# maturk/dn-splatter

Hardware: AMD Instinct MI355X
Metric: fwd+bwd frames/sec @1M Gaussians 1080p; HBM GB/s vs roofline (higher is better)
Workload: dtype f32; 1 GPU; c2: 1000000 random-init Gaussians, 1 camera/GPU 1920x1080, SH degree 3 + expected depth + per-Gaussian normals (7 channels, fused one-pass, post-ops in HIP), fx=fy=1200.0, orbit r=8, closed-form 3-NN scale init, random dense cotangents; scene=reference_init, N=1000000, pixels=2073600, bin_policy=deferred, parallelism=single GPU

## Files before the change

dn-splatter_amd/csrc/binning.hip:

```cpp

#include <assert.h>
#include <string.h>
#include "splat_common.h"
#include "bin_ranges.h"
#include "depth_buckets.h"

namespace {

constexpr int RS_THREADS = 256;
#ifndef DNS_RS_ITEMS_I
#define DNS_RS_ITEMS_I 16
#endif
constexpr int RS_ITEMS_I = DNS_RS_ITEMS_I;
#ifndef DNS_RS_ITEMS_N
#define DNS_RS_ITEMS_N 8
#endif
constexpr int RS_ITEMS_N = DNS_RS_ITEMS_N;
constexpr int RS_ITEMS_N_LARGE = 2 * DNS_RS_ITEMS_N;
constexpr int RS_LARGE_N = 1 << 22;
inline int rs_items_n(int N) { return N >= RS_LARGE_N ? RS_ITEMS_N_LARGE : RS_ITEMS_N; }
#ifndef DNS_TI_THREADS
#define DNS_TI_THREADS 512
#endif
constexpr int TI_THREADS = DNS_TI_THREADS;
// ... 28 lines not shown
#pragma unroll
    for (int i = 0; i < NW; ++i) {
        uint32_t s = lds_wave[i];
        if (i < w) base += s;
        tot += s;
    }
    total = tot;
    __syncthreads();
    return inc + base;
}
__device__ __forceinline__ uint32_t block_incl_scan_256(uint32_t v, uint32_t *lds_wave , uint32_t &total)
{
    return block_incl_scan<4>(v, lds_wave, total);
}

__device__ __forceinline__ uint32_t depth_key(const int32_t *__restrict__ radii, const float *__restrict__ depths, uint32_t g)
{
    return radii[g] > 0 ? __float_as_uint(depths[g]) : 0xFFFFFFFFu;
}

struct __align__(16) EmitRec {
    uint32_t gid;
    uint32_t start;
    uint32_t base_tile;
    uint32_t bw;
};
struct GenArgs {
    const EmitRec *__restrict__ jrec;
    const uint32_t *__restrict__ cum;
    const uint32_t *__restrict__ chunk_first;
// ... 128 lines not shown
                k[i] = __float_as_uint(depths[idc]);
                ok[i] = ok[i] && r > 0;
            } else k[i] = (uint32_t)keys[idc];
        }
#pragma unroll
        for (int i = 0; i < ITEMS; ++i)
            if (ok[i]) atomicAdd(&hist[(k[i] >> shift) & mask], 1u);
    }
    __syncthreads();
    if (threadIdx.x <= mask) table[(size_t)threadIdx.x * nb + blockIdx.x] = hist[threadIdx.x];
}

#ifndef DNS_GEN_HIST_RANGES
#define DNS_GEN_HIST_RANGES 1
#endif
template <int ITEMS, int TH>
__global__ __launch_bounds__(TH) void radix_hist_ranges_kernel(const uint32_t *__restrict__ n_ptr, uint32_t n_cap, int dbits,
                                                               uint32_t *__restrict__ table, int nb, int32_t *__restrict__ tile_first,
                                                               int n_tiles, int32_t *__restrict__ tile_end, GenArgs gen,
                                                               uint32_t *__restrict__ status)
{
    __shared__ uint32_t diff[RS_DIGITS + 1];
    __shared__ uint32_t all_s;
    __shared__ uint32_t lds_wave[TH / DNS_WAVE];
    static_assert(TH > RS_DIGITS, "one thread per difference slot");
    const uint32_t n = n_ptr ? min(*n_ptr, n_cap) : n_cap;
    if (tile_first)
        for (int i = blockIdx.x * TH + threadIdx.x; i <= n_tiles; i += gridDim.x * TH) tile_first[i] = (int32_t)n;
    if (tile_end)
        for (int i = blockIdx.x * TH + threadIdx.x; i < n_tiles; i += gridDim.x * TH) tile_end[i] = 0;
    if (status && blockIdx.x == 0 && threadIdx.x == 0) *status = 0u;
    const uint32_t ND = 1u << dbits;
    if (threadIdx.x <= ND) diff[threadIdx.x] = 0u;
    if (threadIdx.x == 0) all_s = 0u;
    __syncthreads();
    const uint32_t q0 = blockIdx.x * (uint32_t)(TH * ITEMS);
    if (q0 < n) {
        const uint32_t q1 = q0 + min((uint32_t)(TH * ITEMS), n - q0);
        const uint32_t j0 = gen.chunk_first[blockIdx.x];
        const uint32_t n_ranked = min(*gen.n_ranked, (uint32_t)gen.N);
        uint32_t all = 0u;
        for (uint32_t jb = j0;; jb += TH) {
            const uint32_t jj = jb + threadIdx.x;
            bool inside = false;
            if (jj < n_ranked) {
                const uint32_t e = gen.cum[jj], s = jj ? gen.cum[jj - 1] : 0u;
                inside = s < q1;
                if (inside && e > s && e > q0) {
                    const uint4 r = *reinterpret_cast<const uint4 *>(gen.jrec + jj);
                    all += dns_record_digit_ranges(r.z, r.w, (uint32_t)gen.tw, max(s, q0) - s, min(e, q1) - s, dbits,
                                                   [&](uint32_t d0, uint32_t len) {
                                                       atomicAdd(&diff[d0], 1u);
                                                       const uint32_t end = d0 + len;
                                                       if (end <= ND) atomicAdd(&diff[end], 0xFFFFFFFFu);
                                                       else { atomicAdd(&diff[0], 1u); atomicAdd(&diff[end - ND], 0xFFFFFFFFu); }
                                                   });
                }
            }
            if (!__syncthreads_or(inside && threadIdx.x == TH - 1)) break;
        }
        if (all) atomicAdd(&all_s, all);
    }
    __syncthreads();
    const uint32_t v = threadIdx.x < ND ? diff[threadIdx.x] : 0u;
    uint32_t tot;
    const uint32_t inc = block_incl_scan<TH / DNS_WAVE>(v, lds_wave, tot);
    if (threadIdx.x < ND) table[(size_t)threadIdx.x * nb + blockIdx.x] = inc + all_s;
}

constexpr int SC_MAX_SEGS = 8;
__global__ __launch_bounds__(SC_THREADS) void radix_scan_kernel(uint32_t *__restrict__ table, int nb, uint32_t *__restrict__ segsum,
                                                                int segs, int seg_len)
{
    __shared__ uint32_t lds_wave[4];
    const int d = blockIdx.x / segs, sgm = blockIdx.x - d * segs;
    uint32_t *row = table + (size_t)d * nb;
    const int lo = sgm * seg_len, hi = min(nb, lo + seg_len);
    uint32_t carry = 0;
    for (int start = lo; start < hi; start += SC_CHUNK) {
        const int i0 = start + threadIdx.x * SC_ITEMS;
        uint32_t v[SC_ITEMS];
        uint32_t s = 0;
// ... 170 lines not shown
        int2 bx[ITEMS];
#pragma unroll
        for (int r = 0; r < ITEMS; ++r) {
            const uint32_t i = min((uint32_t)(r * TH + threadIdx.x), n_out - 1u);
            const uint32_t d = ((uint32_t)keys_s[i] >> shift) & DMASK;
            dsts[r] = gbase[d] + (i - dstart[d]);
            vs[r] = vals_s[i];
        }
#pragma unroll
        for (int r = 0; r < ITEMS; ++r) bx[r] = box_in[vs[r]];
#pragma unroll
        for (int r = 0; r < ITEMS; ++r)
            if ((uint32_t)(r * TH + threadIdx.x) < n_out) {
                vals_out[dsts[r]] = vs[r];
                box_out[dsts[r]] = bx[r];
                tiles_out[dsts[r]] = ((uint32_t)bx[r].y & 0xffffu) * ((uint32_t)bx[r].y >> 16);
            }
        return;
    }
#pragma unroll
    for (int r = 0; r < ITEMS; ++r) {
        const uint32_t i = r * TH + threadIdx.x;
        if (i < n_out) {
            const uint32_t k = keys_s[i];
            const uint32_t d = (k >> shift) & DMASK;
            const uint32_t dst = gbase[d] + (i - dstart[d]);
            if (!LAST) keys_out[dst] = (K)k;
            vals_out[dst] = vals_s[i];
            if (LAST && (i == 0 || (uint32_t)keys_s[i - 1] != k)) atomicMin(&tile_first[k], (int32_t)dst);
            if (LAST && tile_end && (i + 1 == n_valid || (uint32_t)keys_s[i + 1] != k)) atomicMax(&tile_end[k], (int32_t)dst + 1);
        }
// ... 44 lines not shown
        uint32_t k[U];
#pragma unroll
        for (int u = 0; u < U; ++u) {
            const uint32_t i = min(i0 + u * DP_THREADS, n - 1u);
            r[u] = radii[i];
            k[u] = __float_as_uint(depths[i]);
        }
#pragma unroll
        for (int u = 0; u < U; ++u)
            if (r[u] > 0) { mn = min(mn, k[u]); mx = max(mx, k[u]); }
    }
    dp_block_minmax(mn, mx, red);
    if (threadIdx.x == 0) { part[2 * blockIdx.x] = mn; part[2 * blockIdx.x + 1] = mx; }
}

template <int BBITS>
__global__ __launch_bounds__(DP_THREADS) void depth_part_hist_kernel(const int32_t *__restrict__ radii, const float *__restrict__ depths,
                                                                     uint32_t n, const uint32_t *__restrict__ part, int n_part,
                                                                     uint32_t *__restrict__ ks, uint32_t *__restrict__ table, int nb,
                                                                     int sub)
{
    constexpr int NB = 1 << BBITS;
    __shared__ uint32_t hist[NB];
    __shared__ uint32_t red[2 * DP_NW];
    uint32_t mn = 0xFFFFFFFFu, mx = 0u;
    for (int i = threadIdx.x; i < n_part; i += DP_THREADS) { mn = min(mn, part[2 * i]); mx = max(mx, part[2 * i + 1]); }
    for (int d = threadIdx.x; d < NB; d += DP_THREADS) hist[d] = 0u;
    dp_block_minmax(mn, mx, red);
    uint32_t kmin = 0u;
    int shift = 0;
    if (mn <= mx) { kmin = mn; shift = dns_depth_bucket_shift(mn, mx, BBITS); }
    if (blockIdx.x == 0 && threadIdx.x == 0) { ks[0] = kmin; ks[1] = (uint32_t)shift; }
    for (int c = 0; c < sub; ++c) {
        const uint32_t base = (blockIdx.x * sub + c) * DP_CHUNK;
        if (base >= n) break;
        int32_t r[DP_ITEMS];
        uint32_t k[DP_ITEMS];
#pragma unroll
        for (int i = 0; i < DP_ITEMS; ++i) {
            const uint32_t idc = min(base + i * DP_THREADS + threadIdx.x, n - 1u);
            r[i] = radii[idc];
            k[i] = __float_as_uint(depths[idc]);
        }
#pragma unroll
        for (int i = 0; i < DP_ITEMS; ++i)
            if (base + i * DP_THREADS + threadIdx.x < n && r[i] > 0) atomicAdd(&hist[dns_depth_bucket(k[i], kmin, shift) & (NB - 1)], 1u);
    }
    __syncthreads();
    for (int d = threadIdx.x; d < NB; d += DP_THREADS) table[(size_t)d * nb + blockIdx.x] = hist[d];
}

template <int BBITS>
__global__ __launch_bounds__(DP_THREADS) void depth_part_scatter_kernel(
    const int32_t *__restrict__ radii, const float *__restrict__ depths, uint32_t n, const uint32_t *__restrict__ ks,
    uint2 *__restrict__ pairs_out, const uint32_t *__restrict__ table, const uint32_t *__restrict__ totals, int nb, int segs, int seg_len,
    uint32_t *__restrict__ count_out, uint32_t *__restrict__ bucket_start, int sub)
{
    constexpr int NB = 1 << BBITS;
    constexpr int DPT = NB / DP_THREADS;
    static_assert(NB % DP_THREADS == 0 && DP_CHUNK <= 0xFFFF, "bucket scan layout / 16-bit chunk-local counts");
    __shared__ __align__(4) uint16_t wave_cnt[DP_NW][NB];
    __shared__ uint32_t gbase[NB];
    __shared__ uint32_t lds_wave[DP_NW];
    const uint32_t base0 = blockIdx.x * sub * DP_CHUNK;
    if (base0 >= n) return;
    const uint32_t kmin = ks[0];
    const int shift = (int)ks[1];
    const int w = threadIdx.x / DNS_WAVE;
    const uint32_t lane = lane_id();
    const uint64_t lt_mask = (lane == 0) ? 0ull : (~0ull >> (64 - lane));
    {
// ... 11 lines not shown
                if (sg < my_seg) pre_tab[q] += v;
            }
            tsum += pre_tot[q];
        }
        uint32_t total;
        const uint32_t inc = block_incl_scan<DP_NW>(tsum, lds_wave, total);
        uint32_t run = inc - tsum;
#pragma unroll
        for (int q = 0; q < DPT; ++q) {
            const int d = threadIdx.x * DPT + q;
            gbase[d] = run + pre_tab[q];
            if (blockIdx.x == 0) bucket_start[d] = run;
            run += pre_tot[q];
        }
        if (blockIdx.x == 0 && threadIdx.x == 0) { bucket_start[NB] = total; *count_out = total; }
    }
    for (int c = 0; c < sub; ++c) {
        const uint32_t base = base0 + c * DP_CHUNK;
        if (base >= n) break;
        {
            uint32_t *z = reinterpret_cast<uint32_t *>(&wave_cnt[0][0]);
            for (int i = threadIdx.x; i < DP_NW * NB / 2; i += DP_THREADS) z[i] = 0u;
        }
        __syncthreads();
        const uint32_t wave_start = base + w * (DNS_WAVE * DP_ITEMS);
        uint32_t key[DP_ITEMS];
        int32_t rad[DP_ITEMS];
        uint16_t rnk[DP_ITEMS];
#pragma unroll
        for (int r = 0; r < DP_ITEMS; ++r) {
// ... 90 lines not shown
            for (int q = 0; q < DP_NW; ++q)
                if (q < w) pos += wave_cnt[q][d];
            dst[pos] = p;
        }
        __syncthreads();
        {
            uint32_t s = 0u;
#pragma unroll
            for (int q = 0; q < DP_NW; ++q) { s += wave_cnt[q][threadIdx.x]; wave_cnt[q][threadIdx.x] = 0u; }
            dig_run[threadIdx.x] += s;
        }
        __syncthreads();
    }
}

__device__ __forceinline__ void dp_store_bucket(const uint2 *res, uint32_t s, uint32_t n, uint32_t *__restrict__ vals_out,
                                                const int2 *__restrict__ box_in, int2 *__restrict__ box_out,
                                                uint32_t *__restrict__ tiles_out)
{
    constexpr int U = 4;
    for (uint32_t i0 = threadIdx.x; i0 < n; i0 += U * DP_THREADS) {
        uint32_t v[U];
        int2 bx[U];
#pragma unroll
        for (int u = 0; u < U; ++u) v[u] = res[min(i0 + u * DP_THREADS, n - 1u)].y;
        if (box_in) {
#pragma unroll
            for (int u = 0; u < U; ++u) bx[u] = box_in[v[u]];
        }
#pragma unroll
        for (int u = 0; u < U; ++u) {
            const uint32_t i = i0 + u * DP_THREADS;
            if (i < n) {
                vals_out[s + i] = v[u];
                if (box_in) {
                    box_out[s + i] = bx[u];
                    tiles_out[s + i] = ((uint32_t)bx[u].y & 0xffffu) * ((uint32_t)bx[u].y >> 16);
                }
            }
        }
    }
}

__device__ __forceinline__ void dp_sort_in_lds(const uint2 *__restrict__ in, uint32_t n, uint32_t kmin, int passes, int dbits, uint2 *buf,
                                               uint32_t *dig_start , uint32_t (*wave_cnt)[256] , uint32_t *lds_wave)
{
    constexpr int ITEMS = DP_CAP / DP_THREADS;
    const int w = threadIdx.x / DNS_WAVE;
    const uint32_t lane = lane_id();
    const uint64_t lt_mask = (lane == 0) ? 0ull : (~0ull >> (64 - lane));
    const int ipw = (int)((n + DP_THREADS - 1) / DP_THREADS);
    const uint32_t first = (uint32_t)w * DNS_WAVE * ipw + lane;
    const uint32_t mask = (1u << dbits) - 1u;
    uint2 p[ITEMS];
    uint32_t rnk[ITEMS];
// ... 45 lines not shown
        for (int r = 0; r < ITEMS; ++r)
            if (r < ipw && first + r * DNS_WAVE < n) {
                const uint32_t d = ((p[r].x - kmin) >> sh) & mask;
                buf[dig_start[d] + wave_cnt[w][d] + rnk[r]] = p[r];
            }
        __syncthreads();
        if (pass + 1 < passes) {
#pragma unroll
            for (int r = 0; r < ITEMS; ++r)
                if (r < ipw) p[r] = buf[min(first + r * DNS_WAVE, n - 1u)];
        }
    }
    __syncthreads();
}

__global__ __launch_bounds__(DP_THREADS) void depth_bucket_sort_kernel(const uint32_t *__restrict__ ks,
                                                                       const uint32_t *__restrict__ bucket_start, uint2 *pairs_a,
                                                                       uint2 *pairs_b, uint32_t *__restrict__ vals_out,
                                                                       const int2 *__restrict__ box_in, int2 *__restrict__ box_out,
                                                                       uint32_t *__restrict__ tiles_out)
{
    __shared__ uint2 buf[DP_CAP];
    __shared__ uint32_t dig_run[256];
    __shared__ uint32_t wave_cnt[DP_NW][256];
    __shared__ uint32_t lds_wave[DP_NW];
    const uint32_t s = bucket_start[blockIdx.x], n = bucket_start[blockIdx.x + 1] - s;
    if (n == 0) return;
    const uint32_t kmin = ks[0];
    const int shift = (int)ks[1];
    const int passes = dns_depth_local_passes(shift), dbits = dns_depth_local_bits(shift);
    if (n <= (uint32_t)DP_CAP) {
        dp_sort_in_lds(pairs_a + s, n, kmin, passes, dbits, buf, dig_run, wave_cnt, lds_wave);
        dp_store_bucket(buf, s, n, vals_out, box_in, box_out, tiles_out);
    } else {
        uint2 *src = pairs_a + s, *dst = pairs_b + s;
        for (int p = 0; p < passes; ++p) {
            dp_lsd_pass(src, dst, n, kmin, p * dbits, dbits, dig_run, wave_cnt, lds_wave);
            uint2 *t = src; src = dst; dst = t;
        }
        dp_store_bucket(src, s, n, vals_out, box_in, box_out, tiles_out);
    }
}

template <bool BOXES>
__global__ __launch_bounds__(SC_THREADS) void scan_sums_kernel(int N, const uint32_t *__restrict__ n_ptr,
                                                               const uint32_t *__restrict__ order,
                                                               const int32_t *__restrict__ tiles,
                                                               uint32_t *__restrict__ sums, uint32_t *__restrict__ tiles_sorted,
                                                               const int2 *__restrict__ boxes = nullptr,
                                                               int2 *__restrict__ boxes_sorted = nullptr)
{
    __shared__ uint32_t lds_wave[4];
    const int n = (int)min(*n_ptr, (uint32_t)N);
    const int base = blockIdx.x * SC_CHUNK + threadIdx.x * SC_ITEMS;
    uint32_t s = 0;
    if (blockIdx.x * SC_CHUNK < n) {
        uint32_t o[SC_ITEMS], t[SC_ITEMS];
        [[maybe_unused]] int2 bx[SC_ITEMS];
#pragma unroll
        for (int i = 0; i < SC_ITEMS; ++i) o[i] = order[min(base + i, n - 1)];
#pragma unroll
        for (int i = 0; i < SC_ITEMS; ++i) {
            if (BOXES) {
                bx[i] = boxes[o[i]];
                t[i] = ((uint32_t)bx[i].y & 0xffffu) * ((uint32_t)bx[i].y >> 16);
            } else t[i] = (uint32_t)tiles[o[i]];
        }
#pragma unroll
        for (int i = 0; i < SC_ITEMS; ++i)
            if (base + i < n) {
                s += t[i];
                tiles_sorted[base + i] = t[i];
                if (BOXES) boxes_sorted[base + i] = bx[i];
            }
    }
    uint32_t tot;
    block_incl_scan_256(s, lds_wave, tot);
    if (threadIdx.x == 0) sums[blockIdx.x] = tot;
}

__global__ __launch_bounds__(SC_THREADS) void scan_sums_sorted_kernel(int N, const uint32_t *__restrict__ n_ptr,
                                                                      const uint32_t *__restrict__ tiles_sorted, uint32_t *__restrict__ sums)
{
    __shared__ uint32_t lds_wave[4];
    const int n = (int)min(*n_ptr, (uint32_t)N);
    const int base = blockIdx.x * SC_CHUNK + threadIdx.x * SC_ITEMS;
    uint32_t s = 0;
#pragma unroll
    for (int i = 0; i < SC_ITEMS; ++i)
        if (base + i < n) s += tiles_sorted[base + i];
    uint32_t tot;
    block_incl_scan_256(s, lds_wave, tot);
    if (threadIdx.x == 0) sums[blockIdx.x] = tot;
}

struct EmitPrep {
    EmitRec *__restrict__ jrec;
    uint32_t *__restrict__ chunk_first;
    int nb_chunks, chunk;
    int n_per_cam, tile_size, tw, th;
    const float *__restrict__ means2d;
    const int32_t *__restrict__ radii;
    const float4 *__restrict__ splats;
    const int2 *__restrict__ boxes;
    const int2 *__restrict__ boxes_sorted;
};

__device__ __forceinline__ void emit_record(const EmitPrep &ep, int N, uint32_t j, uint32_t gid, uint32_t start, uint32_t end)
{
    EmitRec r;
    r.gid = gid; r.start = start;
    const uint32_t cam_tiles = (ep.n_per_cam < N) ? (gid / (uint32_t)ep.n_per_cam) * (uint32_t)(ep.tw * ep.th) : 0u;
    if (ep.boxes) {
        const int2 b = ep.boxes_sorted ? ep.boxes_sorted[j] : ep.boxes[gid];
        r.bw = (uint32_t)b.y & 0xffffu;
        r.base_tile = (uint32_t)b.x + cam_tiles;
    } else {
        int x0, y0, x1, y1;
        if (ep.splats) {
            const float4 r0 = ep.splats[(size_t)gid * 4], r1 = ep.splats[(size_t)gid * 4 + 1];
            dns_snug_tile_bbox(r0.x, r0.y, r0.z, r0.w, r1.x, r1.y, (float)ep.radii[gid], ep.tile_size, ep.tw, ep.th, x0, y0, x1, y1);
        } else
            dns_tile_bbox(ep.means2d[2 * gid], ep.means2d[2 * gid + 1], (float)ep.radii[gid], ep.tile_size, ep.tw, ep.th, x0, y0, x1, y1);
        r.base_tile = (uint32_t)(y0 * ep.tw + x0) + cam_tiles;
        r.bw = (uint32_t)(x1 - x0);
    }
    ep.jrec[j] = r;
    const uint32_t c_lo = (start + (uint32_t)ep.chunk - 1u) / (uint32_t)ep.chunk, c_hi = (end - 1u) / (uint32_t)ep.chunk;
    for (uint32_t c = c_lo; c <= c_hi && c < (uint32_t)ep.nb_chunks; ++c) ep.chunk_first[c] = j;
}

__global__ __launch_bounds__(SC_THREADS) void scan_final_kernel(int N, const uint32_t *__restrict__ n_ptr,
                                                                const uint32_t *__restrict__ order,
                                                                const int32_t *__restrict__ tiles,
                                                                const uint32_t *__restrict__ sums,
                                                                uint32_t *__restrict__ cum, uint32_t *__restrict__ total_u32,
                                                                int64_t *__restrict__ total_i64, int64_t *__restrict__ total_max)
{
    __shared__ uint32_t lds_wave[4];
    const int n = (int)min(*n_ptr, (uint32_t)N);
    if (n == 0 && blockIdx.x == 0 && threadIdx.x == 0) { *total_u32 = 0u; *total_i64 = 0; }
    if (blockIdx.x * SC_CHUNK >= n) return;
    const int base = blockIdx.x * SC_CHUNK + threadIdx.x * SC_ITEMS;
    uint32_t v[SC_ITEMS];
// ... 82 lines not shown
    uint32_t *key_a, *key_b, *val_a, *val_b;
    uint32_t *cum;
    uint32_t *tiles_sorted;
    int2 *boxes_sorted;
    EmitRec *jrec;
    uint32_t *chunk_first;
    uint32_t *tab_n;
    uint32_t *totals;
    uint32_t *sums;
    uint32_t *total;
    uint32_t *status;
    uint32_t *n_ranked;
    uint32_t *dp_part;
    uint32_t *dp_ks;
    uint32_t *dp_start;
    uint32_t *dp_tab;
    uint32_t *dp_totals;
    uint32_t *tkey_b, *tval_b;
    uint32_t *tkey_c, *tval_c;
    uint32_t *tab_i;
    int nb_n, nb_i, nb_scan, nb_p;
    size_t bytes;
};

inline size_t align_up(size_t v, size_t a) { return (v + a - 1) / a * a; }

BinWs carve(void *ws, int N, int64_t cap)
{
    BinWs b{};
    b.nb_n = (N + RS_THREADS * rs_items_n(N) - 1) / (RS_THREADS * rs_items_n(N));
    b.nb_i = (int)((cap + RS_THREADS * RS_ITEMS_I - 1) / (RS_THREADS * RS_ITEMS_I));
    b.nb_scan = (N + SC_CHUNK - 1) / SC_CHUNK;
// ... 11 lines not shown
    };
    size_t n = (size_t)(N > 0 ? N : 1), c = (size_t)(cap > 0 ? cap : 1);
    b.key_a = take(n); b.key_b = take(n); b.val_a = take(n); b.val_b = take(n);
    b.cum = take(n);
    b.tiles_sorted = take(n);
    b.boxes_sorted = reinterpret_cast<int2 *>(take(2 * n));
    b.jrec = reinterpret_cast<EmitRec *>(take(4 * n));
    b.chunk_first = take(MAX_CHUNKS);
    b.tab_n = take((size_t)RS_DIGITS * b.nb_n);
    b.totals = take((size_t)RS_DIGITS * SC_MAX_SEGS);
    b.sums = take(b.nb_scan);
    b.total = take(1);
    b.status = take(1);
    b.n_ranked = take(1);
    {
        const size_t B = (size_t)1 << dp_bbits(N), tab = B * b.nb_p;
        uint32_t *q = b.chunk_first;
        b.dp_part = q; q += 2 * DP_BOUNDS_WGS;
        b.dp_ks = q; q += 64;
        b.dp_start = q; q += align_up(B + 1, 64);
        b.dp_totals = q; q += B * SC_MAX_SEGS;
        const bool in_heads = (size_t)(q - b.chunk_first) + tab <= (size_t)MAX_CHUNKS;
        b.dp_tab = in_heads ? q : b.key_a;
        assert((size_t)(q - b.chunk_first) <= (size_t)MAX_CHUNKS && (in_heads || tab <= (size_t)(b.val_a - b.key_a)));
    }
    b.tkey_b = take(c); b.tval_b = take(c);
    b.tkey_c = take(c); b.tval_c = take(c);
    b.tab_i = take((size_t)RS_DIGITS * b.nb_i);
    b.bytes = off;
    return b;
}

int tile_bits(int n_tiles);

template <typename K, int ITEMS, int TH = RS_THREADS>
void radix_pass(hipStream_t stream, const K *ka, const uint32_t *va, K *kb, uint32_t *vb, const uint32_t *n_ptr,
                uint32_t n_cap, int shift, int dbits, uint32_t *table, uint32_t *totals, int nb, int32_t *tile_first = nullptr,
                const int32_t *radii = nullptr, const float *depths = nullptr, int32_t *init_offsets = nullptr, int n_tiles = 0,
                int32_t *tile_end = nullptr, const GenArgs *gen = nullptr, uint32_t *status = nullptr, uint32_t *count_out = nullptr,
                const int2 *box_in = nullptr, int2 *box_out = nullptr, uint32_t *tiles_out = nullptr)
{
    const uint32_t mask = (1u << dbits) - 1u;
    int segs, seg_len;
    scan_segments(nb, segs, seg_len);
    if (radii) {
        hipLaunchKernelGGL((radix_hist_kernel<K, ITEMS, true, false, TH>), dim3(nb), dim3(TH), 0, stream, ka, n_ptr, n_cap, shift, mask, table, nb, radii, depths);
        hipLaunchKernelGGL(radix_scan_kernel, dim3((1 << dbits) * segs), dim3(SC_THREADS), 0, stream, table, nb, totals, segs, seg_len);
        hipLaunchKernelGGL((radix_scatter_kernel<K, false, 8, ITEMS, true, false, TH>), dim3(nb), dim3(TH), 0, stream, ka, va, kb, vb,
                           n_ptr, n_cap, shift, table, totals, nb, tile_first, radii, depths, (int32_t *)nullptr, GenArgs{}, count_out,
                           (const int2 *)nullptr, (int2 *)nullptr, (uint32_t *)nullptr, segs, seg_len);
        return;
    }
    const GenArgs g = gen ? *gen : GenArgs{};
    if (gen && DNS_GEN_HIST_RANGES && shift == 0 && TH > RS_DIGITS)
        hipLaunchKernelGGL((radix_hist_ranges_kernel<ITEMS, (TH > RS_DIGITS ? TH : 2 * RS_DIGITS)>), dim3(nb), dim3(TH), 0, stream, n_ptr, n_cap, dbits,
                           table, nb, init_offsets, n_tiles, init_offsets ? tile_end : nullptr, g, status);
    else if (gen)
        hipLaunchKernelGGL((radix_hist_kernel<K, ITEMS, false, true, TH>), dim3(nb), dim3(TH), 0, stream, ka, n_ptr, n_cap, shift, mask,
                           table, nb, (const int32_t *)nullptr, (const float *)nullptr, init_offsets, n_tiles, init_offsets ? tile_end : nullptr, g, status);
    else
        hipLaunchKernelGGL((radix_hist_kernel<K, ITEMS, false, false, TH>), dim3(nb), dim3(TH), 0, stream, ka, n_ptr, n_cap, shift, mask, table, nb,
                           (const int32_t *)nullptr, (const float *)nullptr, init_offsets, n_tiles, init_offsets ? tile_end : nullptr, g, status);
    hipLaunchKernelGGL(radix_scan_kernel, dim3((1 << dbits) * segs), dim3(SC_THREADS), 0, stream, table, nb, totals, segs, seg_len);
    if constexpr (sizeof(K) == 4) {
        if (box_in && !gen && !tile_first && dbits == 8) {
            hipLaunchKernelGGL((radix_scatter_kernel<K, false, 8, ITEMS, false, false, TH, true>), dim3(nb), dim3(TH), 0, stream, ka, va, kb, vb,
                               n_ptr, n_cap, shift, table, totals, nb, tile_first, (const int32_t *)nullptr, (const float *)nullptr,
                               (int32_t *)nullptr, GenArgs{}, (uint32_t *)nullptr, box_in, box_out, tiles_out, segs, seg_len);
            return;
        }
    }
// ... 195 lines not shown
    BinWs w = carve(a->workspace, a->N, a->isect_capacity);
    const int N = a->N;
    if (a->tight_tiles && !a->splats && !a->tile_boxes && N > 0) return DNSPLAT_ERR_INVALID_ARG;
    if (N == 0) {
        if (hipMemsetAsync(a->n_isects, 0, sizeof(int64_t), stream) != hipSuccess) return DNSPLAT_ERR_LAUNCH;
        if (hipMemsetAsync(w.total, 0, sizeof(uint32_t), stream) != hipSuccess) return DNSPLAT_ERR_LAUNCH;
    } else {
        const uint32_t n_u32 = (uint32_t)N;
        uint32_t *ka = w.key_a, *kb = w.key_b, *va = w.val_a, *vb = w.val_b;
        const int2 *boxes = reinterpret_cast<const int2 *>(a->tile_boxes);
        static const bool box_gather = [] { const char *e = getenv("DNSPLAT_BIN_BOX_GATHER"); return !(e && e[0] == '0'); }();
        const bool sorted_boxes = boxes && box_gather;
        static const bool box_fold = [] { const char *e = getenv("DNSPLAT_BIN_BOX_FOLD"); return !(e && e[0] == '0'); }();
        const bool fold = sorted_boxes && box_fold;
        const bool radix4 = !depth_sort_by_partition(N);
        if (!radix4) {
            uint2 *pairs_a = reinterpret_cast<uint2 *>(w.jrec), *pairs_b = pairs_a + N;
            const int n_part = dp_bounds_wgs(N), sub = dp_sub(N);
            int segs, seg_len;
            scan_segments(w.nb_p, segs, seg_len);
            hipLaunchKernelGGL(depth_bounds_kernel, dim3(n_part), dim3(DP_THREADS), 0, stream, a->radii, a->depths, n_u32, w.dp_part);
#define DNS_DEPTH_PARTITION(B)                                                                                                            \
    do {                                                                                                                                  \
        hipLaunchKernelGGL(depth_part_hist_kernel<B>, dim3(w.nb_p), dim3(DP_THREADS), 0, stream, a->radii, a->depths, n_u32, w.dp_part,   \
                           n_part, w.dp_ks, w.dp_tab, w.nb_p, sub);                                                                       \
        hipLaunchKernelGGL(radix_scan_kernel, dim3((1 << B) * segs), dim3(SC_THREADS), 0, stream, w.dp_tab, w.nb_p, w.dp_totals, segs,    \
                           seg_len);                                                                                                      \
        hipLaunchKernelGGL(depth_part_scatter_kernel<B>, dim3(w.nb_p), dim3(DP_THREADS), 0, stream, a->radii, a->depths, n_u32, w.dp_ks,  \
                           pairs_a, w.dp_tab, w.dp_totals, w.nb_p, segs, seg_len, w.n_ranked, w.dp_start, sub);                           \
    } while (0)
            const int bbits = dp_bbits(N);
            switch (bbits) {
                case 9: DNS_DEPTH_PARTITION(9); break;
                case 10: DNS_DEPTH_PARTITION(10); break;
                case 11: DNS_DEPTH_PARTITION(11); break;
                default: DNS_DEPTH_PARTITION(12); break;
            }
#undef DNS_DEPTH_PARTITION
            hipLaunchKernelGGL(depth_bucket_sort_kernel, dim3(1 << bbits), dim3(DP_THREADS), 0, stream, w.dp_ks, w.dp_start, pairs_a, pairs_b,
                               w.val_a, fold ? boxes : nullptr, w.boxes_sorted, w.tiles_sorted);
        } else {
            for (int pass = 0; pass < 4; ++pass) {
                const int shift = 8 * pass;
                const bool fold_here = fold && pass == 3;
                if (rs_items_n(N) == RS_ITEMS_N_LARGE)
                    radix_pass<uint32_t, RS_ITEMS_N_LARGE>(stream, ka, va, kb, vb, pass == 0 ? nullptr : w.n_ranked, n_u32, shift, 8, w.tab_n, w.totals,
                                                           w.nb_n, nullptr, pass == 0 ? a->radii : nullptr, pass == 0 ? a->depths : nullptr, nullptr, 0,
                                                           nullptr, nullptr, nullptr, pass == 0 ? w.n_ranked : nullptr,
                                                           fold_here ? boxes : nullptr, w.boxes_sorted, w.tiles_sorted);
                else
                    radix_pass<uint32_t, RS_ITEMS_N>(stream, ka, va, kb, vb, pass == 0 ? nullptr : w.n_ranked, n_u32, shift, 8, w.tab_n, w.totals,
                                                     w.nb_n, nullptr, pass == 0 ? a->radii : nullptr, pass == 0 ? a->depths : nullptr, nullptr, 0,
                                                     nullptr, nullptr, nullptr, pass == 0 ? w.n_ranked : nullptr,
                                                     fold_here ? boxes : nullptr, w.boxes_sorted, w.tiles_sorted);
                uint32_t *t = ka; ka = kb; kb = t;
                t = va; va = vb; vb = t;
            }
        }
        if (fold)
            hipLaunchKernelGGL(scan_sums_sorted_kernel, dim3(w.nb_scan), dim3(SC_THREADS), 0, stream, N, w.n_ranked, w.tiles_sorted, w.sums);
        else if (sorted_boxes)
            hipLaunchKernelGGL(scan_sums_kernel<true>, dim3(w.nb_scan), dim3(SC_THREADS), 0, stream, N, w.n_ranked, w.val_a, a->tiles_per_gauss,
                               w.sums, w.tiles_sorted, boxes, w.boxes_sorted);
        else
            hipLaunchKernelGGL(scan_sums_kernel<false>, dim3(w.nb_scan), dim3(SC_THREADS), 0, stream, N, w.n_ranked, w.val_a, a->tiles_per_gauss,
                               w.sums, w.tiles_sorted);
        EmitPrep ep;
        ep.jrec = w.jrec; ep.chunk_first = w.chunk_first; ep.nb_chunks = MAX_CHUNKS; ep.chunk = RS_THREADS * RS_ITEMS_I;
        ep.n_per_cam = N / (a->n_cameras > 1 ? a->n_cameras : 1);
        ep.tile_size = a->tile_size;
        ep.tw = dns_tiles_w(a->width, a->tile_size); ep.th = dns_tiles_h(a->height, a->tile_size);
        ep.means2d = a->means2d; ep.radii = a->radii;
        ep.splats = a->tight_tiles ? reinterpret_cast<const float4 *>(a->splats) : nullptr;
        ep.boxes = boxes;
        ep.boxes_sorted = sorted_boxes ? w.boxes_sorted : nullptr;
        hipLaunchKernelGGL(scan_final_kernel, dim3(w.nb_scan), dim3(SC_THREADS), 0, stream, N, w.n_ranked, w.val_a,
                           (const int32_t *)w.tiles_sorted, w.sums, w.cum, w.total, a->n_isects, a->n_isects_max);
        hipLaunchKernelGGL(emit_prep_kernel, dim3((N + 255) / 256), dim3(256), 0, stream, N, w.n_ranked, w.val_a, w.cum, ep);
        DNS_CHECK_LAUNCH();
    }
    if (a->n_isects_host) {
        if (hipMemcpyAsync(a->n_isects_host, a->n_isects, sizeof(int64_t), hipMemcpyDeviceToHost, stream) != hipSuccess)
            return DNSPLAT_ERR_LAUNCH;
    }
    return DNSPLAT_OK;
}

extern "C" int dnsplat_bin_emit_sort(const dnsplat_bin_args *a, dnsplat_stream_t stream_)
{
    int rc = check_bin(a);
    if (rc != DNSPLAT_OK) return rc;
    if (!a->tile_offsets || (a->isect_capacity > 0 && !a->flatten_ids)) return DNSPLAT_ERR_INVALID_ARG;
    if (a->tight_tiles && !a->splats && !a->tile_boxes && a->N > 0) return DNSPLAT_ERR_INVALID_ARG;
// ... 36 lines not shown
```

Baseline: 486.1 frames/s.

## Fuse tile-count prefix scan and emit-record prep into depth bucket sort

The depth-partition histogram now also accumulates per-bucket tile-pair sums, and the scatter kernel scans them into per-bucket pair starts. The bucket sort kernel then computes cumulative tile offsets and writes emit records directly. This drops the separate scan_sums, scan_final and emit_prep kernels and their extra passes over sorted arrays. The range histogram kernel also now runs with a configurable, smaller thread count by giving each thread several digits. Costs are extra LDS atomics in the histogram and a serial per-bucket scan inside the sort blocks.

```diff
diff --git a/dn-splatter_amd/csrc/binning.hip b/dn-splatter_amd/csrc/binning.hip
--- a/dn-splatter_amd/csrc/binning.hip
+++ b/dn-splatter_amd/csrc/binning.hip
@@ -66,6 +66,8 @@
     return block_incl_scan<4>(v, lds_wave, total);
 }
 
+__device__ __forceinline__ uint32_t dns_box_tiles(const int2 b) { return ((uint32_t)b.y & 0xffffu) * ((uint32_t)b.y >> 16); }
+
 __device__ __forceinline__ uint32_t depth_key(const int32_t *__restrict__ radii, const float *__restrict__ depths, uint32_t g)
 {
     return radii[g] > 0 ? __float_as_uint(depths[g]) : 0xFFFFFFFFu;
@@ -224,6 +226,10 @@
 #ifndef DNS_GEN_HIST_RANGES
 #define DNS_GEN_HIST_RANGES 1
 #endif
+#ifndef DNS_HR_THREADS
+#define DNS_HR_THREADS 256
+#endif
+constexpr int HR_THREADS = DNS_HR_THREADS;
 template <int ITEMS, int TH>
 __global__ __launch_bounds__(TH) void radix_hist_ranges_kernel(const uint32_t *__restrict__ n_ptr, uint32_t n_cap, int dbits,
                                                                uint32_t *__restrict__ table, int nb, int32_t *__restrict__ tile_first,
@@ -233,7 +239,8 @@
     __shared__ uint32_t diff[RS_DIGITS + 1];
     __shared__ uint32_t all_s;
     __shared__ uint32_t lds_wave[TH / DNS_WAVE];
-    static_assert(TH > RS_DIGITS, "one thread per difference slot");
+    constexpr int PER = (RS_DIGITS + TH - 1) / TH;
+    static_assert(TH % DNS_WAVE == 0 && TH >= DNS_WAVE, "whole waves");
     const uint32_t n = n_ptr ? min(*n_ptr, n_cap) : n_cap;
     if (tile_first)
         for (int i = blockIdx.x * TH + threadIdx.x; i <= n_tiles; i += gridDim.x * TH) tile_first[i] = (int32_t)n;
@@ -241,7 +248,7 @@
         for (int i = blockIdx.x * TH + threadIdx.x; i < n_tiles; i += gridDim.x * TH) tile_end[i] = 0;
     if (status && blockIdx.x == 0 && threadIdx.x == 0) *status = 0u;
     const uint32_t ND = 1u << dbits;
-    if (threadIdx.x <= ND) diff[threadIdx.x] = 0u;
+    for (uint32_t d = threadIdx.x; d <= ND; d += TH) diff[d] = 0u;
     if (threadIdx.x == 0) all_s = 0u;
     __syncthreads();
     const uint32_t q0 = blockIdx.x * (uint32_t)(TH * ITEMS);
@@ -272,10 +279,22 @@
         if (all) atomicAdd(&all_s, all);
     }
     __syncthreads();
-    const uint32_t v = threadIdx.x < ND ? diff[threadIdx.x] : 0u;
+    uint32_t v[PER];
+    uint32_t sum = 0u;
+#pragma unroll
+    for (int p = 0; p < PER; ++p) {
+        const uint32_t d = threadIdx.x * PER + p;
+        v[p] = d < ND ? diff[d] : 0u;
+        sum += v[p];
+    }
     uint32_t tot;
-    const uint32_t inc = block_incl_scan<TH / DNS_WAVE>(v, lds_wave, tot);
-    if (threadIdx.x < ND) table[(size_t)threadIdx.x * nb + blockIdx.x] = inc + all_s;
+    uint32_t run = block_incl_scan<TH / DNS_WAVE>(sum, lds_wave, tot) - sum + all_s;
+#pragma unroll
+    for (int p = 0; p < PER; ++p) {
+        const uint32_t d = threadIdx.x * PER + p;
+        run += v[p];
+        if (d < ND) table[(size_t)d * nb + blockIdx.x] = run;
+    }
 }
 
 constexpr int SC_MAX_SEGS = 8;
@@ -476,7 +495,7 @@
             if ((uint32_t)(r * TH + threadIdx.x) < n_out) {
                 vals_out[dsts[r]] = vs[r];
                 box_out[dsts[r]] = bx[r];
-                tiles_out[dsts[r]] = ((uint32_t)bx[r].y & 0xffffu) * ((uint32_t)bx[r].y >> 16);
+                tiles_out[dsts[r]] = dns_box_tiles(bx[r]);
             }
         return;
     }
@@ -551,18 +570,22 @@
     if (threadIdx.x == 0) { part[2 * blockIdx.x] = mn; part[2 * blockIdx.x + 1] = mx; }
 }
 
-template <int BBITS>
+template <int BBITS, bool PAIRS>
 __global__ __launch_bounds__(DP_THREADS) void depth_part_hist_kernel(const int32_t *__restrict__ radii, const float *__restrict__ depths,
                                                                      uint32_t n, const uint32_t *__restrict__ part, int n_part,
                                                                      uint32_t *__restrict__ ks, uint32_t *__restrict__ table, int nb,
-                                                                     int sub)
+                                                                     int sub, const int2 *__restrict__ boxes)
 {
     constexpr int NB = 1 << BBITS;
     __shared__ uint32_t hist[NB];
+    __shared__ uint32_t psum[PAIRS ? NB : 1];
     __shared__ uint32_t red[2 * DP_NW];
     uint32_t mn = 0xFFFFFFFFu, mx = 0u;
     for (int i = threadIdx.x; i < n_part; i += DP_THREADS) { mn = min(mn, part[2 * i]); mx = max(mx, part[2 * i + 1]); }
-    for (int d = threadIdx.x; d < NB; d += DP_THREADS) hist[d] = 0u;
+    for (int d = threadIdx.x; d < NB; d += DP_THREADS) {
+        hist[d] = 0u;
+        if (PAIRS) psum[d] = 0u;
+    }
     dp_block_minmax(mn, mx, red);
     uint32_t kmin = 0u;
     int shift = 0;
@@ -573,25 +596,42 @@
         if (base >= n) break;
         int32_t r[DP_ITEMS];
         uint32_t k[DP_ITEMS];
+        [[maybe_unused]] int2 bx[DP_ITEMS];
 #pragma unroll
         for (int i = 0; i < DP_ITEMS; ++i) {
             const uint32_t idc = min(base + i * DP_THREADS + threadIdx.x, n - 1u);
             r[i] = radii[idc];
             k[i] = __float_as_uint(depths[idc]);
+            if (PAIRS) bx[i] = boxes[idc];
         }
 #pragma unroll
         for (int i = 0; i < DP_ITEMS; ++i)
-            if (base + i * DP_THREADS + threadIdx.x < n && r[i] > 0) atomicAdd(&hist[dns_depth_bucket(k[i], kmin, shift) & (NB - 1)], 1u);
-    }
-    __syncthreads();
-    for (int d = threadIdx.x; d < NB; d += DP_THREADS) table[(size_t)d * nb + blockIdx.x] = hist[d];
-}
-
-template <int BBITS>
+            if (base + i * DP_THREADS + threadIdx.x < n && r[i] > 0) {
+                const uint32_t d = dns_depth_bucket(k[i], kmin, shift) & (NB - 1);
+                atomicAdd(&hist[d], 1u);
+                if (PAIRS) {
+                    const uint32_t t = dns_box_tiles(bx[i]);
+                    if (t) atomicAdd(&psum[d], t);
+                }
+            }
+    }
+    __syncthreads();
+    for (int d = threadIdx.x; d < NB; d += DP_THREADS) {
+        table[(size_t)d * nb + blockIdx.x] = hist[d];
+        if (PAIRS) table[(size_t)(NB + d) * nb + blockIdx.x] = psum[d];
+    }
+}
+
+struct PairTotals {
+    uint32_t *__restrict__ pair_start;
+    uint32_t *__restrict__ total_u32;
+    int64_t *__restrict__ total_i64, *__restrict__ total_max;
+};
+template <int BBITS, bool PAIRS>
 __global__ __launch_bounds__(DP_THREADS) void depth_part_scatter_kernel(
     const int32_t *__restrict__ radii, const float *__restrict__ depths, uint32_t n, const uint32_t *__restrict__ ks,
     uint2 *__restrict__ pairs_out, const uint32_t *__restrict__ table, const uint32_t *__restrict__ totals, int nb, int segs, int seg_len,
-    uint32_t *__restrict__ count_out, uint32_t *__restrict__ bucket_start, int sub)
+    uint32_t *__restrict__ count_out, uint32_t *__restrict__ bucket_start, int sub, PairTotals pt)
 {
     constexpr int NB = 1 << BBITS;
     constexpr int DPT = NB / DP_THREADS;
@@ -633,6 +673,30 @@
             run += pre_tot[q];
         }
         if (blockIdx.x == 0 && threadIdx.x == 0) { bucket_start[NB] = total; *count_out = total; }
+        if (PAIRS && blockIdx.x == 0) {
+            uint32_t ptot[DPT];
+            uint32_t psum = 0u;
+#pragma unroll
+            for (int q = 0; q < DPT; ++q) {
+                const int d = NB + threadIdx.x * DPT + q;
+                ptot[q] = 0u;
+                for (int sg = 0; sg < segs; ++sg) ptot[q] += totals[d * segs + sg];
+                psum += ptot[q];
+            }
+            uint32_t ptotal;
+            const uint32_t pinc = block_incl_scan<DP_NW>(psum, lds_wave, ptotal);
+            uint32_t prun = pinc - psum;
+#pragma unroll
+            for (int q = 0; q < DPT; ++q) {
+                pt.pair_start[threadIdx.x * DPT + q] = prun;
+                prun += ptot[q];
+            }
+            if (threadIdx.x == 0) {
+                pt.pair_start[NB] = ptotal;
+                *pt.total_u32 = ptotal; *pt.total_i64 = (int64_t)ptotal;
+                if (pt.total_max) atomicMax(reinterpret_cast<unsigned long long *>(pt.total_max), (unsigned long long)ptotal);
+            }
+        }
     }
     for (int c = 0; c < sub; ++c) {
         const uint32_t base = base0 + c * DP_CHUNK;
@@ -753,6 +817,43 @@
     }
 }
 
+struct EmitPrep {
+    EmitRec *__restrict__ jrec;
+    uint32_t *__restrict__ chunk_first;
+    int nb_chunks, chunk;
+    int n_per_cam, tile_size, tw, th;
+    const float *__restrict__ means2d;
+    const int32_t *__restrict__ radii;
+    const float4 *__restrict__ splats;
+    const int2 *__restrict__ boxes;
+    const int2 *__restrict__ boxes_sorted;
+};
+
+__device__ __forceinline__ void emit_record(const EmitPrep &ep, int N, uint32_t j, uint32_t gid, uint32_t start, uint32_t end,
+                                            const int2 *box = nullptr)
+{
+    EmitRec r;
+    r.gid = gid; r.start = start;
+    const uint32_t cam_tiles = (ep.n_per_cam < N) ? (gid / (uint32_t)ep.n_per_cam) * (uint32_t)(ep.tw * ep.th) : 0u;
+    if (ep.boxes) {
+        const int2 b = box ? *box : ep.boxes_sorted ? ep.boxes_sorted[j] : ep.boxes[gid];
+        r.bw = (uint32_t)b.y & 0xffffu;
+        r.base_tile = (uint32_t)b.x + cam_tiles;
+    } else {
+        int x0, y0, x1, y1;
+        if (ep.splats) {
+            const float4 r0 = ep.splats[(size_t)gid * 4], r1 = ep.splats[(size_t)gid * 4 + 1];
+            dns_snug_tile_bbox(r0.x, r0.y, r0.z, r0.w, r1.x, r1.y, (float)ep.radii[gid], ep.tile_size, ep.tw, ep.th, x0, y0, x1, y1);
+        } else
+            dns_tile_bbox(ep.means2d[2 * gid], ep.means2d[2 * gid + 1], (float)ep.radii[gid], ep.tile_size, ep.tw, ep.th, x0, y0, x1, y1);
+        r.base_tile = (uint32_t)(y0 * ep.tw + x0) + cam_tiles;
+        r.bw = (uint32_t)(x1 - x0);
+    }
+    ep.jrec[j] = r;
+    const uint32_t c_lo = (start + (uint32_t)ep.chunk - 1u) / (uint32_t)ep.chunk, c_hi = (end - 1u) / (uint32_t)ep.chunk;
+    for (uint32_t c = c_lo; c <= c_hi && c < (uint32_t)ep.nb_chunks; ++c) ep.chunk_first[c] = j;
+}
+
 __device__ __forceinline__ void dp_store_bucket(const uint2 *res, uint32_t s, uint32_t n, uint32_t *__restrict__ vals_out,
                                                 const int2 *__restrict__ box_in, int2 *__restrict__ box_out,
                                                 uint32_t *__restrict__ tiles_out)
@@ -774,10 +875,56 @@
                 vals_out[s + i] = v[u];
                 if (box_in) {
                     box_out[s + i] = bx[u];
-                    tiles_out[s + i] = ((uint32_t)bx[u].y & 0xffffu) * ((uint32_t)bx[u].y >> 16);
+                    tiles_out[s + i] = dns_box_tiles(bx[u]);
                 }
             }
         }
+    }
+}
+
+__device__ __forceinline__ void dp_emit_bucket(const uint2 *res, uint32_t s, uint32_t n, uint32_t pbase, uint32_t *__restrict__ vals_out,
+                                               const int2 *__restrict__ box_in, uint32_t *__restrict__ cum, const EmitPrep &ep, int N,
+                                               uint32_t *lds_wave )
+{
+    constexpr int U = 4;
+    const int w = threadIdx.x / DNS_WAVE;
+    uint32_t carry = pbase;
+    for (uint32_t b0 = 0; b0 < n; b0 += U * DP_THREADS) {
+        const uint32_t i0 = b0 + (uint32_t)w * (DNS_WAVE * U) + lane_id();
+        uint32_t v[U], t[U], inc[U];
+        int2 bx[U];
+#pragma unroll
+        for (int u = 0; u < U; ++u) v[u] = res[min(i0 + u * DNS_WAVE, n - 1u)].y;
+#pragma unroll
+        for (int u = 0; u < U; ++u) bx[u] = box_in[v[u]];
+        uint32_t wave_tot = 0u;
+#pragma unroll
+        for (int u = 0; u < U; ++u) {
+            t[u] = i0 + u * DNS_WAVE < n ? dns_box_tiles(bx[u]) : 0u;
+            inc[u] = wave_incl_scan(t[u]) + wave_tot;
+            wave_tot = __shfl(inc[u], DNS_WAVE - 1, DNS_WAVE);
+        }
+        if (lane_id() == DNS_WAVE - 1) lds_wave[w] = wave_tot;
+        __syncthreads();
+        uint32_t before = carry, tot = 0u;
+#pragma unroll
+        for (int i = 0; i < DP_NW; ++i) {
+            const uint32_t ws = lds_wave[i];
+            if (i < w) before += ws;
+            tot += ws;
+        }
+        __syncthreads();
+#pragma unroll
+        for (int u = 0; u < U; ++u) {
+            const uint32_t i = i0 + u * DNS_WAVE;
+            if (i < n) {
+                const uint32_t end = before + inc[u];
+                vals_out[s + i] = v[u];
+                cum[s + i] = end;
+                if (t[u]) emit_record(ep, N, s + i, v[u], end - t[u], end, &bx[u]);
+            }
+        }
+        carry += tot;
     }
 }
 
@@ -853,11 +1000,17 @@
     __syncthreads();
 }
 
+#ifndef DNS_DP_FUSED_EMIT
+#define DNS_DP_FUSED_EMIT 1
+#endif
+template <bool EMIT>
 __global__ __launch_bounds__(DP_THREADS) void depth_bucket_sort_kernel(const uint32_t *__restrict__ ks,
                                                                        const uint32_t *__restrict__ bucket_start, uint2 *pairs_a,
                                                                        uint2 *pairs_b, uint32_t *__restrict__ vals_out,
                                                                        const int2 *__restrict__ box_in, int2 *__restrict__ box_out,
-                                                                       uint32_t *__restrict__ tiles_out)
+                                                                       uint32_t *__restrict__ tiles_out,
+                                                                       const uint32_t *__restrict__ pair_start, uint32_t *__restrict__ cum,
+                                                                       EmitPrep ep, int N)
 {
     __shared__ uint2 buf[DP_CAP];
     __shared__ uint32_t dig_run[256];
@@ -870,14 +1023,16 @@
     const int passes = dns_depth_local_passes(shift), dbits = dns_depth_local_bits(shift);
     if (n <= (uint32_t)DP_CAP) {
         dp_sort_in_lds(pairs_a + s, n, kmin, passes, dbits, buf, dig_run, wave_cnt, lds_wave);
-        dp_store_bucket(buf, s, n, vals_out, box_in, box_out, tiles_out);
+        if (EMIT) dp_emit_bucket(buf, s, n, pair_start[blockIdx.x], vals_out, box_in, cum, ep, N, lds_wave);
+        else dp_store_bucket(buf, s, n, vals_out, box_in, box_out, tiles_out);
     } else {
         uint2 *src = pairs_a + s, *dst = pairs_b + s;
         for (int p = 0; p < passes; ++p) {
             dp_lsd_pass(src, dst, n, kmin, p * dbits, dbits, dig_run, wave_cnt, lds_wave);
             uint2 *t = src; src = dst; dst = t;
         }
-        dp_store_bucket(src, s, n, vals_out, box_in, box_out, tiles_out);
+        if (EMIT) dp_emit_bucket(src, s, n, pair_start[blockIdx.x], vals_out, box_in, cum, ep, N, lds_wave);
+        else dp_store_bucket(src, s, n, vals_out, box_in, box_out, tiles_out);
     }
 }
 
@@ -902,7 +1057,7 @@
         for (int i = 0; i < SC_ITEMS; ++i) {
             if (BOXES) {
                 bx[i] = boxes[o[i]];
-                t[i] = ((uint32_t)bx[i].y & 0xffffu) * ((uint32_t)bx[i].y >> 16);
+                t[i] = dns_box_tiles(bx[i]);
             } else t[i] = (uint32_t)tiles[o[i]];
         }
 #pragma unroll
@@ -931,42 +1086,6 @@
     uint32_t tot;
     block_incl_scan_256(s, lds_wave, tot);
     if (threadIdx.x == 0) sums[blockIdx.x] = tot;
-}
-
-struct EmitPrep {
-    EmitRec *__restrict__ jrec;
-    uint32_t *__restrict__ chunk_first;
-    int nb_chunks, chunk;
-    int n_per_cam, tile_size, tw, th;
-    const float *__restrict__ means2d;
-    const int32_t *__restrict__ radii;
-    const float4 *__restrict__ splats;
-    const int2 *__restrict__ boxes;
-    const int2 *__restrict__ boxes_sorted;
-};
-
-__device__ __forceinline__ void emit_record(const EmitPrep &ep, int N, uint32_t j, uint32_t gid, uint32_t start, uint32_t end)
-{
-    EmitRec r;
-    r.gid = gid; r.start = start;
-    const uint32_t cam_tiles = (ep.n_per_cam < N) ? (gid / (uint32_t)ep.n_per_cam) * (uint32_t)(ep.tw * ep.th) : 0u;
-    if (ep.boxes) {
-        const int2 b = ep.boxes_sorted ? ep.boxes_sorted[j] : ep.boxes[gid];
-        r.bw = (uint32_t)b.y & 0xffffu;
-        r.base_tile = (uint32_t)b.x + cam_tiles;
-    } else {
-        int x0, y0, x1, y1;
-        if (ep.splats) {
-            const float4 r0 = ep.splats[(size_t)gid * 4], r1 = ep.splats[(size_t)gid * 4 + 1];
-            dns_snug_tile_bbox(r0.x, r0.y, r0.z, r0.w, r1.x, r1.y, (float)ep.radii[gid], ep.tile_size, ep.tw, ep.th, x0, y0, x1, y1);
-        } else
-            dns_tile_bbox(ep.means2d[2 * gid], ep.means2d[2 * gid + 1], (float)ep.radii[gid], ep.tile_size, ep.tw, ep.th, x0, y0, x1, y1);
-        r.base_tile = (uint32_t)(y0 * ep.tw + x0) + cam_tiles;
-        r.bw = (uint32_t)(x1 - x0);
-    }
-    ep.jrec[j] = r;
-    const uint32_t c_lo = (start + (uint32_t)ep.chunk - 1u) / (uint32_t)ep.chunk, c_hi = (end - 1u) / (uint32_t)ep.chunk;
-    for (uint32_t c = c_lo; c <= c_hi && c < (uint32_t)ep.nb_chunks; ++c) ep.chunk_first[c] = j;
 }
 
 __global__ __launch_bounds__(SC_THREADS) void scan_final_kernel(int N, const uint32_t *__restrict__ n_ptr,
@@ -1079,8 +1198,10 @@
     uint32_t *dp_part;
     uint32_t *dp_ks;
     uint32_t *dp_start;
+    uint32_t *dp_pair_start;
     uint32_t *dp_tab;
     uint32_t *dp_totals;
+    bool dp_fused_ok;
     uint32_t *tkey_b, *tval_b;
     uint32_t *tkey_c, *tval_c;
     uint32_t *tab_i;
@@ -1122,15 +1243,19 @@
     b.status = take(1);
     b.n_ranked = take(1);
     {
-        const size_t B = (size_t)1 << dp_bbits(N), tab = B * b.nb_p;
+        const size_t B = (size_t)1 << dp_bbits(N), tab = 2 * B * b.nb_p, starts = align_up(B + 1, 64);
         uint32_t *q = b.chunk_first;
         b.dp_part = q; q += 2 * DP_BOUNDS_WGS;
-        b.dp_ks = q; q += 64;
-        b.dp_start = q; q += align_up(B + 1, 64);
-        b.dp_totals = q; q += B * SC_MAX_SEGS;
+        b.dp_totals = q; q += 2 * B * SC_MAX_SEGS;
+        uint32_t *safe = 64 + 2 * starts <= (size_t)RS_DIGITS * SC_MAX_SEGS ? b.totals
+                       : 64 + 2 * starts <= (size_t)(b.cum - b.val_b)        ? b.val_b
+                                                                             : nullptr;
+        b.dp_fused_ok = safe != nullptr;
+        if (!safe) { safe = q; q += 64 + 2 * starts; }
+        b.dp_ks = safe; b.dp_start = safe + 64; b.dp_pair_start = b.dp_start + starts;
         const bool in_heads = (size_t)(q - b.chunk_first) + tab <= (size_t)MAX_CHUNKS;
-        b.dp_tab = in_heads ? q : b.key_a;
-        assert((size_t)(q - b.chunk_first) <= (size_t)MAX_CHUNKS && (in_heads || tab <= (size_t)(b.val_a - b.key_a)));
+        b.dp_tab = in_heads ? q : b.tiles_sorted;
+        assert((size_t)(q - b.chunk_first) <= (size_t)MAX_CHUNKS && (in_heads || tab <= (size_t)((uint32_t *)b.boxes_sorted - b.tiles_sorted)));
     }
     b.tkey_b = take(c); b.tval_b = take(c);
     b.tkey_c = take(c); b.tval_c = take(c);
@@ -1160,9 +1285,12 @@
         return;
     }
     const GenArgs g = gen ? *gen : GenArgs{};
-    if (gen && DNS_GEN_HIST_RANGES && shift == 0 && TH > RS_DIGITS)
-        hipLaunchKernelGGL((radix_hist_ranges_kernel<ITEMS, (TH > RS_DIGITS ? TH : 2 * RS_DIGITS)>), dim3(nb), dim3(TH), 0, stream, n_ptr, n_cap, dbits,
+    if (gen && DNS_GEN_HIST_RANGES && shift == 0) {
+        constexpr int HR_ITEMS = TH * ITEMS / HR_THREADS;
+        static_assert(HR_THREADS * HR_ITEMS == TH * ITEMS, "the range histogram counts the scatter's chunks");
+        hipLaunchKernelGGL((radix_hist_ranges_kernel<HR_ITEMS, HR_THREADS>), dim3(nb), dim3(HR_THREADS), 0, stream, n_ptr, n_cap, dbits,
                            table, nb, init_offsets, n_tiles, init_offsets ? tile_end : nullptr, g, status);
+    }
     else if (gen)
         hipLaunchKernelGGL((radix_hist_kernel<K, ITEMS, false, true, TH>), dim3(nb), dim3(TH), 0, stream, ka, n_ptr, n_cap, shift, mask,
                            table, nb, (const int32_t *)nullptr, (const float *)nullptr, init_offsets, n_tiles, init_offsets ? tile_end : nullptr, g, status);
@@ -1388,20 +1516,37 @@
         static const bool box_fold = [] { const char *e = getenv("DNSPLAT_BIN_BOX_FOLD"); return !(e && e[0] == '0'); }();
         const bool fold = sorted_boxes && box_fold;
         const bool radix4 = !depth_sort_by_partition(N);
+        EmitPrep ep;
+        ep.jrec = w.jrec; ep.chunk_first = w.chunk_first; ep.nb_chunks = MAX_CHUNKS; ep.chunk = RS_THREADS * RS_ITEMS_I;
+        ep.n_per_cam = N / (a->n_cameras > 1 ? a->n_cameras : 1);
+        ep.tile_size = a->tile_size;
+        ep.tw = dns_tiles_w(a->width, a->tile_size); ep.th = dns_tiles_h(a->height, a->tile_size);
+        ep.means2d = a->means2d; ep.radii = a->radii;
+        ep.splats = a->tight_tiles ? reinterpret_cast<const float4 *>(a->splats) : nullptr;
+        ep.boxes = boxes;
+        ep.boxes_sorted = sorted_boxes ? w.boxes_sorted : nullptr;
+        const bool fused_emit = DNS_DP_FUSED_EMIT && !radix4 && fold && w.dp_fused_ok;
         if (!radix4) {
-            uint2 *pairs_a = reinterpret_cast<uint2 *>(w.jrec), *pairs_b = pairs_a + N;
+            uint2 *pairs_a = reinterpret_cast<uint2 *>(fused_emit ? (void *)w.key_a : (void *)w.jrec);
+            uint2 *pairs_b = fused_emit ? reinterpret_cast<uint2 *>(w.boxes_sorted) : pairs_a + N;
             const int n_part = dp_bounds_wgs(N), sub = dp_sub(N);
             int segs, seg_len;
             scan_segments(w.nb_p, segs, seg_len);
+            const PairTotals pt{w.dp_pair_start, w.total, a->n_isects, a->n_isects_max};
             hipLaunchKernelGGL(depth_bounds_kernel, dim3(n_part), dim3(DP_THREADS), 0, stream, a->radii, a->depths, n_u32, w.dp_part);
+#define DNS_DEPTH_PARTITION2(B, P)                                                                                                        \
+    do {                                                                                                                                  \
+        hipLaunchKernelGGL((depth_part_hist_kernel<B, P>), dim3(w.nb_p), dim3(DP_THREADS), 0, stream, a->radii, a->depths, n_u32,         \
+                           w.dp_part, n_part, w.dp_ks, w.dp_tab, w.nb_p, sub, boxes);                                                     \
+        hipLaunchKernelGGL(radix_scan_kernel, dim3(((P ? 2 : 1) << B) * segs), dim3(SC_THREADS), 0, stream, w.dp_tab, w.nb_p,             \
+                           w.dp_totals, segs, seg_len);                                                                                   \
+        hipLaunchKernelGGL((depth_part_scatter_kernel<B, P>), dim3(w.nb_p), dim3(DP_THREADS), 0, stream, a->radii, a->depths, n_u32,      \
+                           w.dp_ks, pairs_a, w.dp_tab, w.dp_totals, w.nb_p, segs, seg_len, w.n_ranked, w.dp_start, sub, pt);              \
+    } while (0)
 #define DNS_DEPTH_PARTITION(B)                                                                                                            \
     do {                                                                                                                                  \
-        hipLaunchKernelGGL(depth_part_hist_kernel<B>, dim3(w.nb_p), dim3(DP_THREADS), 0, stream, a->radii, a->depths, n_u32, w.dp_part,   \
-                           n_part, w.dp_ks, w.dp_tab, w.nb_p, sub);                                                                       \
-        hipLaunchKernelGGL(radix_scan_kernel, dim3((1 << B) * segs), dim3(SC_THREADS), 0, stream, w.dp_tab, w.nb_p, w.dp_totals, segs,    \
-                           seg_len);                                                                                                      \
-        hipLaunchKernelGGL(depth_part_scatter_kernel<B>, dim3(w.nb_p), dim3(DP_THREADS), 0, stream, a->radii, a->depths, n_u32, w.dp_ks,  \
-                           pairs_a, w.dp_tab, w.dp_totals, w.nb_p, segs, seg_len, w.n_ranked, w.dp_start, sub);                           \
+        if (fused_emit) DNS_DEPTH_PARTITION2(B, true);                                                                                    \
+        else DNS_DEPTH_PARTITION2(B, false);                                                                                              \
     } while (0)
             const int bbits = dp_bbits(N);
             switch (bbits) {
@@ -1411,8 +1556,14 @@
                 default: DNS_DEPTH_PARTITION(12); break;
             }
 #undef DNS_DEPTH_PARTITION
-            hipLaunchKernelGGL(depth_bucket_sort_kernel, dim3(1 << bbits), dim3(DP_THREADS), 0, stream, w.dp_ks, w.dp_start, pairs_a, pairs_b,
-                               w.val_a, fold ? boxes : nullptr, w.boxes_sorted, w.tiles_sorted);
+#undef DNS_DEPTH_PARTITION2
+            if (fused_emit)
+                hipLaunchKernelGGL(depth_bucket_sort_kernel<true>, dim3(1 << bbits), dim3(DP_THREADS), 0, stream, w.dp_ks, w.dp_start, pairs_a,
+                                   pairs_b, w.val_a, boxes, (int2 *)nullptr, (uint32_t *)nullptr, w.dp_pair_start, w.cum, ep, N);
+            else
+                hipLaunchKernelGGL(depth_bucket_sort_kernel<false>, dim3(1 << bbits), dim3(DP_THREADS), 0, stream, w.dp_ks, w.dp_start, pairs_a,
+                                   pairs_b, w.val_a, fold ? boxes : nullptr, w.boxes_sorted, w.tiles_sorted, (const uint32_t *)nullptr,
+                                   (uint32_t *)nullptr, ep, N);
         } else {
             for (int pass = 0; pass < 4; ++pass) {
                 const int shift = 8 * pass;
@@ -1431,7 +1582,8 @@
                 t = va; va = vb; vb = t;
             }
         }
-        if (fold)
+        if (fused_emit) {}
+        else if (fold)
             hipLaunchKernelGGL(scan_sums_sorted_kernel, dim3(w.nb_scan), dim3(SC_THREADS), 0, stream, N, w.n_ranked, w.tiles_sorted, w.sums);
         else if (sorted_boxes)
             hipLaunchKernelGGL(scan_sums_kernel<true>, dim3(w.nb_scan), dim3(SC_THREADS), 0, stream, N, w.n_ranked, w.val_a, a->tiles_per_gauss,
@@ -1439,18 +1591,11 @@
         else
             hipLaunchKernelGGL(scan_sums_kernel<false>, dim3(w.nb_scan), dim3(SC_THREADS), 0, stream, N, w.n_ranked, w.val_a, a->tiles_per_gauss,
                                w.sums, w.tiles_sorted);
-        EmitPrep ep;
-        ep.jrec = w.jrec; ep.chunk_first = w.chunk_first; ep.nb_chunks = MAX_CHUNKS; ep.chunk = RS_THREADS * RS_ITEMS_I;
-        ep.n_per_cam = N / (a->n_cameras > 1 ? a->n_cameras : 1);
-        ep.tile_size = a->tile_size;
-        ep.tw = dns_tiles_w(a->width, a->tile_size); ep.th = dns_tiles_h(a->height, a->tile_size);
-        ep.means2d = a->means2d; ep.radii = a->radii;
-        ep.splats = a->tight_tiles ? reinterpret_cast<const float4 *>(a->splats) : nullptr;
-        ep.boxes = boxes;
-        ep.boxes_sorted = sorted_boxes ? w.boxes_sorted : nullptr;
-        hipLaunchKernelGGL(scan_final_kernel, dim3(w.nb_scan), dim3(SC_THREADS), 0, stream, N, w.n_ranked, w.val_a,
-                           (const int32_t *)w.tiles_sorted, w.sums, w.cum, w.total, a->n_isects, a->n_isects_max);
-        hipLaunchKernelGGL(emit_prep_kernel, dim3((N + 255) / 256), dim3(256), 0, stream, N, w.n_ranked, w.val_a, w.cum, ep);
+        if (!fused_emit) {
+            hipLaunchKernelGGL(scan_final_kernel, dim3(w.nb_scan), dim3(SC_THREADS), 0, stream, N, w.n_ranked, w.val_a,
+                               (const int32_t *)w.tiles_sorted, w.sums, w.cum, w.total, a->n_isects, a->n_isects_max);
+            hipLaunchKernelGGL(emit_prep_kernel, dim3((N + 255) / 256), dim3(256), 0, stream, N, w.n_ranked, w.val_a, w.cum, ep);
+        }
         DNS_CHECK_LAUNCH();
     }
     if (a->n_isects_host) {
```

Result: no change. 487.5 frames/s, median of 2 (+0.3%).
